# yuliangguo/OmniFusion

Measured on AMD Instinct MI355X. Metric: panoramas/sec at 512x1024 ERP, N=18 256^2 patches; equi2pers+pers2equi GB/s vs HBM peak, higher is better.
Workload: dtype f16x3 (fp16 hi/lo pairs, fp32 accumulate: fp32-class); 1 GPU; cfg2/cfg4 shard: 8 panoramas/GPU/step, 512x1024 ERP, fov 80, nrows 4 (18 patches); full single-pass spherical_fusion forward (confidence=True) at patch size 128 — the only size the reference network exists at (SURVEY 0.1); random-init weights (seed 42); inputs resident in HBM; resample pair at 18x256^2 reported in roofline_resample; per_gpu_batch=8, global_batch=8, parallelism=image-sharded x1, execution=3 forwards in flight per GPU on 3 streams (spherical_fusion.pipelined)

## Files before the change

include/omnifusion.h:

```cpp
#ifndef OMNIFUSION_H_
#define OMNIFUSION_H_

#include <stddef.h>
#include <stdint.h>

#ifdef __cplusplus
extern "C" {
#endif

#define OMNI_VERSION 200

enum omni_status {
    OMNI_OK = 0,
    OMNI_ERR_INVALID = 1,
    OMNI_ERR_HIP = 2,
    OMNI_ERR_UNSUPPORTED = 3
};

enum omni_layout { OMNI_LAYOUT_BCHWN = 0, OMNI_LAYOUT_BNCHW = 1, OMNI_LAYOUT_BNHWC = 2,
                   OMNI_LAYOUT_BCHNW = 3  };
enum omni_dtype { OMNI_F32 = 0, OMNI_F16 = 1 };

typedef void* omni_stream_t;
typedef struct omni_geometry omni_geometry_t;
// ... 42 lines not shown
                       int ph, int pw, int nrows, float fov_h, float fov_w, int layout, omni_stream_t stream);
int omni_pers2equi_bwd(const void* grad_erp, void* grad_pers, int dtype, int B, int C, int ph, int pw,
                       int H, int W, int nrows, float fov_h, float fov_w, int layout, omni_stream_t stream);
int omni_conv2d_nhwc_f32(const float* src1, const float* src2, const float* wt, const float* bias,
                         const float* res, float* dst, int M, int H, int W, int C1, int C2, int Cout,
                         int KH, int KW, int stride, int pad, int act, omni_stream_t stream);
int omni_conv2d_splitk_plan(long long rows, int Cout, int ksteps);
int omni_conv2d_nhwc_f32_ws(const float* src1, const float* src2, const float* wt, const float* bias,
                            const float* res, float* dst, int M, int H, int W, int C1, int C2, int Cout,
                            int KH, int KW, int stride, int pad, int act, int splitk, float* ws, size_t ws_bytes,
                            omni_stream_t stream);
int omni_conv2d_nhwc_f16x3_ws(const float* src1, const float* src2, const void* wt16, const float* bias,
                              const float* res, float* dst, int M, int H, int W, int C1, int C2, int Cout,
                              int KH, int KW, int stride, int pad, int act, int splitk, float* ws, size_t ws_bytes,
                              omni_stream_t stream);
int omni_conv2d_sh_f16x3_ws(const void* src1, const void* src2, const void* wt16, const float* bias,
                            const void* res, void* dst, int fmt, int M, int H, int W, int C1, int C2, int Cout,
                            int KH, int KW, int stride, int pad, int act, int splitk, float* ws, size_t ws_bytes,
                            omni_stream_t stream);
int omni_gemm_rows_sh_f16x3(const void* x, const void* wt16r, const float* bias, const float* res, void* dst, int fmt,
                            int rows, int K, int N, int act, omni_stream_t stream);
int omni_gemm_rows_pack(const void* wt16, void* wt16r, int N, int K, omni_stream_t stream);
int omni_gemm_rows_ln_sh_f16x3(const float* x, const float* ln_weight, const float* ln_bias, float eps, const void* wt16r, const float* bias,
                               const float* res, void* dst, int fmt, int rows, int N, int act, omni_stream_t stream);
int omni_conv3x3_up2_sh_f16x3(const void* src, const void* wt16, const float* bias, void* dst, int fmt,
                              int M, int Hl, int Wl, int C, int Cout, int act, omni_stream_t stream);
size_t omni_up2_heads_scratch_bytes(int M, int P);
int omni_conv3x3_up2_heads_sh_f16x3(const void* src, const void* wt16, const float* bias, const void* heads_w16f, float bias_pred, float bias_weight,
                                    float* scratch, size_t scratch_bytes, float* out_a, float* out_c, int M, int P, int confidence, omni_stream_t stream);
int omni_conv3x3_up2_heads_sh_f16x1(const void* src, const void* wt16, const float* bias, const void* heads_w16f, float bias_pred, float bias_weight,
                                    float* scratch, size_t scratch_bytes, float* out_a, float* out_c, int M, int P, int confidence, omni_stream_t stream);
int omni_heads_pack_f16x3(const float* w_host, void* dst_host);
int omni_conv2d_sh_f16x3_post_ws(const void* src1, const void* src2, const void* wt16, const float* bias,
                                 const void* res, void* dst, int fmt, int M, int H, int W, int C1, int C2, int Cout,
                                 int KH, int KW, int stride, int pad, int act, int splitk, float* ws, size_t ws_bytes,
                                 const float* post, size_t post_elems, omni_stream_t stream);
int omni_wino_input_sh(const void* src, void* V, int M, int H, int W, int C, omni_stream_t stream);
int omni_conv3x3_wino_sh_f16x3(const void* V, const void* wt16, const float* bias, const void* res, void* dst, int fmt,
                               int M, int H, int W, int C, int Cout, int act, int splitk, float* ws, size_t ws_bytes, omni_stream_t stream);
int omni_sh_from_f32(const float* src, void* dst, size_t n, omni_stream_t stream);
int omni_sh_to_f32(const void* src, float* dst, size_t n, omni_stream_t stream);
int omni_sh_overflow(int* flag, int reset);
int omni_stem_f32(const float* src, const float* wt, const float* bias, float* dst, int M, int P, omni_stream_t stream);
int omni_maxpool3x3s2_f32(const float* src, float* dst, int M, int H, int W, int C, omni_stream_t stream);
int omni_upsample_bilinear_f32(const float* src, float* dst, int M, int H, int W, int C, int Ho, int Wo, omni_stream_t stream);
int omni_add_hw_f32(float* x, const float* y, int M, int HW, int C, omni_stream_t stream);
int omni_add_period_f32(float* x, const float* y, size_t total, size_t period, omni_stream_t stream);
int omni_stem_sh(const float* src, const float* wt, const float* bias, void* dst, int M, int P, omni_stream_t stream);
int omni_stem_sh_f16x3(const float* src, const void* wt16, const float* bias, void* dst, int M, int P, omni_stream_t stream);
int omni_stem_sh_f16x1(const float* src, const void* wt16, const float* bias, void* dst, int M, int P, omni_stream_t stream);
int omni_maxpool3x3s2_sh(const void* src, void* dst, int M, int H, int W, int C, omni_stream_t stream);
int omni_upsample_bilinear_sh(const void* src, void* dst, int M, int H, int W, int C, int Ho, int Wo, omni_stream_t stream);
int omni_up2_tapsum_sh(const float* y, const float* bias, void* dst, int M, int Hl, int Wl, int Cout, int act, omni_stream_t stream);
int omni_add_hw_sh(void* x, const float* y, int M, int HW, int C, omni_stream_t stream);
int omni_add_period_sh(void* x, const float* y, size_t total, size_t period, omni_stream_t stream);
int omni_layernorm512_sh(const float* x, const float* g, const float* b, void* y, int rows, float eps, omni_stream_t stream);
int omni_gemm_rows_slices_sh_f16x3(const void* x, const void* wt16r, float* parts, int rows, int K, int N, int slices, omni_stream_t stream);
int omni_gemm_rows_ln_parts_sh_f16x3(const float* parts, int nparts, const float* pbias, const float* pres, float* xout,
                                     const float* ln_weight, const float* ln_bias, float eps, const void* wt16r, const float* bias,
                                     void* dst, int fmt, int rows, int N, int act, omni_stream_t stream);
int omni_splitk_reduce_ln512(const float* parts, int nparts, const float* bias, const float* res, float* tok, const float* ln_weight, const float* ln_bias,
                             float eps, void* y, int fmt, int rows, omni_stream_t stream);
int omni_gemm_sh_f16x3_ln512_ws(const void* x, const void* wt16, const float* bias, const float* res, float* tok, const float* ln_g, const float* ln_b,
                                float eps, void* y, int fmt, int rows, int K, int splitk, float* ws, size_t ws_bytes, omni_stream_t stream);
int omni_attention_qkv_sh(const float* qkv, void* out, int B, int N, omni_stream_t stream);
int omni_token_pack_f32(const float* d, const float* pos, float* tok, int M, int N, int HW, int C, omni_stream_t stream);
int omni_layernorm512_f32(const float* x, const float* g, const float* b, float* y, int rows, float eps, omni_stream_t stream);
int omni_attention_f32(const float* q, const float* kv, float* out, int B, int N, omni_stream_t stream);
int omni_heads_f32(const float* x, const float* w, float bias_pred, float bias_weight, float* out_a, float* out_c,
                   int M, int P, int confidence, omni_stream_t stream);
int omni_mlp_points_f32(const float* xyz, const float* depth, const float* w1, const float* b1, const float* w2,
                        const float* b2, float* out, int Mo, int N, int HW, omni_stream_t stream);

int omni_masked_median_f32(const float* x, const float* mask, size_t n, unsigned* ws, float* out, omni_stream_t stream);
int omni_depth_metrics_f32(float* pred, const float* gt, const float* mask, const float* scale_num, const float* scale_den,
                           size_t n, double* ws, float* out, omni_stream_t stream);

size_t omni_semantic_workspace_bytes(size_t npix);
int omni_semantic_step_f32(const float* logits, const int64_t* target, int B, int C, size_t HW, int64_t ignore_index, int K,
                           void* workspace, float* loss, int64_t* pred, int64_t* confusion, omni_stream_t stream);
int omni_semantic_grad_f32(const float* logits, const int64_t* target, int B, int C, size_t HW, int64_t ignore_index,
                           const void* workspace, const float* grad_out, float* grad_logits, omni_stream_t stream);
int omni_confusion_matrix_i64(const int64_t* pred, const int64_t* gt, size_t n, int K, int64_t* confusion, int64_t* n_bad,
                              omni_stream_t stream);

int omni_preprocess_rgb_u8(const unsigned char* src_hwc, float* dst_chw, int B, int Hs, int Ws, int H, int W, omni_stream_t stream);
int omni_preprocess_depth_u16(const unsigned short* src, float* depth, unsigned char* mask, int B, int Hs, int Ws, int H, int W,
                              float min_depth, float max_depth, omni_stream_t stream);
int omni_png_info(const void* data, size_t nbytes, int* width, int* height, int* bit_depth, int* color_type);
int omni_png_decode(const void* data, size_t nbytes, void* dst, int H, int W, int kind);
int omni_png_decode_batch(const void* const* datas, const size_t* nbytes, void* const* dsts, int n, int H, int W, int kind, int threads);
int omni_zlib_inflate(const void* src, size_t nbytes, void* dst, size_t cap, size_t* produced, size_t* consumed);
int omni_png_checksums(const void* data, size_t nbytes, unsigned* crc32, unsigned* adler32);
size_t omni_berhu_workspace_bytes(int B);
int omni_berhu_loss_f32(const float* pred, const float* gt, const float* mask, const float* weights, int B, size_t per_item,
                        void* workspace, float* loss, omni_stream_t stream);
int omni_berhu_grad_f32(const float* pred, const float* gt, const float* mask, const float* weights, int B, size_t per_item,
                        const void* workspace, const float* grad_out, float* grad_pred, omni_stream_t stream);
int omni_pointcloud_ply_f32(const float* depth, const float* rgb, unsigned char* records, int B, int H, int W, omni_stream_t stream);

size_t omni_dibr_workspace_bytes(int B, int C, int H, int W);
int omni_splat_render_f32(const float* img, const float* depth, const float* coords, float max_depth,
                          float* recon, unsigned char* mask , int B, int C, int H, int W,
                          void* workspace, omni_stream_t stream);
int omni_dibr_f32(const float* img, const float* depth, const float* uvgrid, const float* sgrid, int grid_batched,
                  float baseline, int mode, float* recon, unsigned char* mask ,
// ... 47 lines not shown
```

omnifusion_amd/_lib.py:

```python
import ctypes
import os

_HERE = os.path.dirname(os.path.abspath(__file__))
LIB_PATH = os.environ.get("OMNI_LIB_VARIANT") or os.path.join(_HERE, "csrc", "libomnifusion_hip.so")
LIB_PATH_DEBUG = os.path.join(_HERE, "csrc", "libomnifusion_hip_dbg.so")

OMNI_OK, OMNI_ERR_INVALID, OMNI_ERR_HIP, OMNI_ERR_UNSUPPORTED = 0, 1, 2, 3
LAYOUT_BCHWN, LAYOUT_BNCHW, LAYOUT_BNHWC, LAYOUT_BCHNW = 0, 1, 2, 3
F32, F16 = 0, 1

_lib = None


class OmniLibraryMissing(ImportError):
    pass


EXPORTS = [
    "omni_version", "omni_last_error", "omni_set_option", "omni_get_option", "omni_num_patches", "omni_patch_centers",
    "omni_geometry_create", "omni_geometry_destroy", "omni_geometry_cache_clear", "omni_geometry_cache_size",
    "omni_equi2pers", "omni_equi2pers_aux", "omni_pers2equi", "omni_pers2equi_conf", "omni_patches_to_planar",
    "omni_equi2pers_g", "omni_pers2equi_g", "omni_equi2pers_bwd", "omni_pers2equi_bwd",
    "omni_conv2d_nhwc_f32", "omni_stem_f32", "omni_maxpool3x3s2_f32", "omni_upsample_bilinear_f32",
    "omni_add_hw_f32", "omni_add_period_f32", "omni_token_pack_f32", "omni_layernorm512_f32",
    "omni_attention_f32", "omni_heads_f32", "omni_mlp_points_f32",
    "omni_conv2d_nhwc_f16x3_ws", "omni_conv2d_sh_f16x3_ws", "omni_conv2d_sh_f16x3_post_ws", "omni_gemm_rows_sh_f16x3", "omni_gemm_rows_ln_sh_f16x3", "omni_gemm_rows_pack", "omni_conv3x3_up2_sh_f16x3", "omni_conv3x3_up2_heads_sh_f16x3", "omni_conv3x3_up2_heads_sh_f16x1", "omni_up2_heads_scratch_bytes", "omni_heads_pack_f16x3", "omni_sh_from_f32", "omni_sh_to_f32", "omni_sh_overflow",
    "omni_stem_sh", "omni_stem_sh_f16x3", "omni_stem_sh_f16x1", "omni_maxpool3x3s2_sh", "omni_upsample_bilinear_sh", "omni_up2_tapsum_sh", "omni_add_hw_sh", "omni_add_period_sh", "omni_layernorm512_sh", "omni_gemm_sh_f16x3_ln512_ws", "omni_gemm_rows_slices_sh_f16x3", "omni_gemm_rows_ln_parts_sh_f16x3", "omni_splitk_reduce_ln512", "omni_wino_input_sh", "omni_conv3x3_wino_sh_f16x3", "omni_attention_qkv_sh",
    "omni_conv2d_splitk_plan", "omni_conv2d_nhwc_f32_ws",
    "omni_masked_median_f32", "omni_depth_metrics_f32",
    "omni_png_info", "omni_png_decode", "omni_png_decode_batch", "omni_zlib_inflate", "omni_png_checksums",
    "omni_preprocess_rgb_u8", "omni_preprocess_depth_u16", "omni_berhu_workspace_bytes", "omni_berhu_loss_f32", "omni_berhu_grad_f32",
    "omni_pointcloud_ply_f32",
    "omni_dibr_workspace_bytes", "omni_splat_render_f32", "omni_dibr_f32",
    "omni_splat_render_wt_f32", "omni_dibr_wt_f32", "omni_dibr_bwd_workspace_bytes", "omni_splat_render_bwd_f32", "omni_dibr_bwd_f32",
    "omni_ssim_f32", "omni_photometric_workspace_bytes", "omni_photometric_grad_scratch_bytes", "omni_photometric_loss_f32",
    "omni_photometric_grad_f32",
    "omni_freeview_rotations", "omni_freeview_equi2pers_f32", "omni_freeview_pers2equi_f32", "omni_freeview_merge_f32",
    "omni_freeview_bwd_workspace_bytes", "omni_freeview_equi2pers_bwd_f32", "omni_freeview_pers2equi_bwd_f32", "omni_freeview_merge_bwd_f32",
    "omni_semantic_workspace_bytes", "omni_semantic_step_f32", "omni_semantic_grad_f32", "omni_confusion_matrix_i64",
]


def load():
    global _lib
    if _lib is not None:
        return _lib
    if not os.path.exists(LIB_PATH):
        raise OmniLibraryMissing(
            f"{LIB_PATH} not found: build it with `python -m omnifusion_amd.build` "
            "(hipcc --offload-arch=gfx950).  There is no fallback path.")
    import torch
    lib = ctypes.CDLL(LIB_PATH)
    lib.omni_last_error.restype = ctypes.c_char_p
    lib.omni_version.restype = ctypes.c_int
    lib.omni_up2_heads_scratch_bytes.restype = ctypes.c_size_t
    lib.omni_dibr_workspace_bytes.restype = ctypes.c_size_t
    lib.omni_splat_render_f32.argtypes = [ctypes.c_void_p] * 3 + [ctypes.c_float] + [ctypes.c_void_p] * 2 + [ctypes.c_int] * 4 + [ctypes.c_void_p] * 2
    lib.omni_dibr_f32.argtypes = [ctypes.c_void_p] * 4 + [ctypes.c_int, ctypes.c_float, ctypes.c_int] + [ctypes.c_void_p] * 2 + \
        [ctypes.c_int] * 4 + [ctypes.c_void_p] * 2
    vp, ci, cf = ctypes.c_void_p, ctypes.c_int, ctypes.c_float
    lib.omni_splat_render_wt_f32.argtypes = [vp] * 3 + [cf] + [vp] * 3 + [ci] * 4 + [vp] * 2
    lib.omni_dibr_wt_f32.argtypes = [vp] * 4 + [ci, cf, ci] + [vp] * 3 + [ci] * 4 + [vp] * 2
    lib.omni_dibr_bwd_workspace_bytes.restype = ctypes.c_size_t
    lib.omni_splat_render_bwd_f32.argtypes = [vp] * 6 + [cf] + [vp] * 3 + [ci] * 4 + [vp] * 2
    lib.omni_dibr_bwd_f32.argtypes = [vp] * 7 + [ci, cf, ci] + [vp] * 2 + [ci] * 4 + [vp] * 2
    lib.omni_ssim_f32.argtypes = [vp] * 2 + [ci] * 5 + [vp, ci, vp, vp]
    lib.omni_photometric_workspace_bytes.restype = ctypes.c_size_t
    lib.omni_photometric_grad_scratch_bytes.restype = ctypes.c_size_t
    lib.omni_photometric_loss_f32.argtypes = [vp, vp, vp, ci, vp, ci] + [ci] * 5 + [vp, ci, cf] + [vp] * 3
    lib.omni_photometric_grad_f32.argtypes = [vp, vp, vp, ci, vp, ci] + [ci] * 5 + [vp, ci, cf] + [vp] * 5
    lib.omni_freeview_rotations.argtypes = [vp, vp, ci, vp, vp]
    lib.omni_freeview_equi2pers_f32.argtypes = [vp] * 3 + [ci] * 7 + [cf, cf, ci, vp]
    lib.omni_freeview_pers2equi_f32.argtypes = [vp] * 4 + [ci] * 6 + [cf, cf, vp]
    lib.omni_freeview_merge_f32.argtypes = [vp] * 4 + [ci] * 7 + [cf, cf, vp]
    lib.omni_freeview_bwd_workspace_bytes.restype = ctypes.c_size_t
    lib.omni_freeview_bwd_workspace_bytes.argtypes = [ci] * 5
    lib.omni_freeview_equi2pers_bwd_f32.argtypes = [vp] * 3 + [ci] * 7 + [cf, cf, ci, vp, vp]
    lib.omni_freeview_pers2equi_bwd_f32.argtypes = [vp] * 3 + [ci] * 6 + [cf, cf, vp, vp]
    lib.omni_freeview_merge_bwd_f32.argtypes = [vp] * 3 + [ci] * 7 + [cf, cf, vp, vp]
    sz, i64 = ctypes.c_size_t, ctypes.c_int64
# ... 63 lines not shown
```

omnifusion_amd/csrc/omni_conv_sh.hip:

```cpp
#include "omni_conv_sh_common.h"

namespace {

__constant__ float wino_coef[16][4] = {
    {1, 0, 0, 0}, {1, 1, 0, 0}, {1, -1, 0, 0}, {0, -1, 0, 0},
    {1, 0, 1, 0}, {1, 1, 1, 1}, {1, -1, 1, -1}, {0, -1, 0, -1},
    {1, 0, -1, 0}, {1, 1, -1, -1}, {1, -1, -1, 1}, {0, -1, 0, 1},
    {0, 0, -1, 0}, {0, 0, -1, -1}, {0, 0, -1, 1}, {0, 0, 0, 1}};
template <int BM, int BN, int WM, int WN, int NST = 3, int NL = 0, bool PP = false, bool WINO = false, bool X1 = false>
__global__ __launch_bounds__(64 * (WM * WN + NL)) void conv_sh_kernel(ShConvArgs a)
{
    static_assert(!(WINO && X1), "Winograd: f16x3 only");
    static_assert(!PP || (NL > 0 && WM * WN == 8 && NST >= 3), "ping-pong: eight matrix waves (two per SIMD) + loader waves, three stages");
    static_assert(!WINO || (PP && BM / WM == 32 && BN / WN == 32), "Winograd: the ping-pong kernel with 32 x 32 wave tiles");
    constexpr int NW = WM * WN, LW = NL > 0 ? NL : NW, RPP = 8 * LW;
    constexpr int TM = BM / WM / 32, TN = BN / WN / 32;
    constexpr int APASS = BM / RPP, BPASS = BN / RPP, LPS = APASS + BPASS;
    static_assert(APASS >= 1 && BPASS >= 1, "a tile side must cover at least one DMA pass");
    constexpr int A_BYTES = BM * 128, STAGE = (BM + BN) * 128;
    __shared__ __attribute__((aligned(1024))) unsigned char lds[NST * STAGE];
    __shared__ long long cst[OMNI_ABL(32768) ? 256 : 1];
    const bool stamped = OMNI_ABL(32768) && blockIdx.x == 0 && blockIdx.y == 0 && a.ws != nullptr && a.splitk <= 1;
    auto cstamp = [&](int k) { if (OMNI_ABL(32768) && stamped && (threadIdx.x & 63) == 0 && k < 256) cst[k] = clock64(); };
    auto cdump = [&]() { if (OMNI_ABL(32768) && stamped && threadIdx.x == 0) for (int i = 0; i < 256; ++i) reinterpret_cast<long long*>(a.ws)[i] = cst[i]; };
// ... 602 lines not shown
    const long long rows = (long long)M * a.Ho * a.Wo;
    if (rows <= 0 || rows >= (1ll << 31) || (long long)M * H * W >= (1ll << 31))
        OMNI_FAIL(OMNI_ERR_UNSUPPORTED, "omni_conv2d_sh: too many pixels for 32-bit row indices");
    a.rows = (int)rows;
    const int ksteps = KH * KW * ((C1 + C2) / 32);
    if ((long long)M * H * W * (C1 > C2 ? C1 : C2) * 4 >= (1ll << 31) || (long long)Cout * ksteps * 128 >= (1ll << 31))
        OMNI_FAIL(OMNI_ERR_UNSUPPORTED, "omni_conv2d_sh: an operand of 2 GiB or more (32-bit buffer offsets)");
    int S = splitk;
    if (S > ksteps) S = ksteps;
    if (S > 1 && (!ws || ws_bytes < (size_t)S * rows * Cout * sizeof(float)))
        OMNI_FAIL(OMNI_ERR_INVALID, "omni_conv2d_sh: split-K workspace too small");
    a.splitk = S > 1 ? S : 1; a.ws = ws;
    a.wt_major = omni_options().conv_wt_major == 2 || (omni_options().conv_wt_major == 1 &&
                 (long long)Cout * ksteps * 128 > (long long)M * H * W * (C1 + C2) * 4) ? 1 : 0;
    a.post = post; a.post_rows = 1; a.wino_th = a.wino_tw = a.wino_pix = 0;
    if (post) {
        if (Cout <= 0 || post_elems == 0 || post_elems % (size_t)Cout || post_elems / (size_t)Cout > 0x7fffffffull)
            OMNI_FAIL(OMNI_ERR_INVALID, "omni_conv2d_sh: the post-activation addend must hold whole rows of Cout channels");
        if (a.splitk > 1) OMNI_FAIL(OMNI_ERR_UNSUPPORTED, "omni_conv2d_sh: no post-activation addend with split-K");
        a.post_rows = (unsigned)(post_elems / (size_t)Cout);
    }
    hipStream_t s = (hipStream_t)stream;
    if (fmt & 8) conv_sh_select<true>(a, fmt, s);
    else         conv_sh_select<false>(a, fmt, s);
    OMNI_HIP(hipGetLastError());
    if (a.splitk > 1 && reduce) {
        const size_t n4 = (size_t)rows * Cout / 4;
        hipLaunchKernelGGL(sh_splitk_reduce_kernel, dim3((unsigned)((n4 + 255) / 256)), dim3(256), 0, s, (const float*)ws, bias, res, dst,
                           n4, Cout, a.splitk, (size_t)rows * Cout, act, a.dst_sh, a.res_f32);
        OMNI_HIP(hipGetLastError());
    }
    return OMNI_OK;
}

extern "C" int omni_splitk_reduce_ln512(const float* parts, int nparts, const float* bias, const float* res, float* tok, const float* lg, const float* lb,
                                        float eps, void* y, int fmt, int rows, omni_stream_t stream)
{
    if (!parts || nparts < 1 || !tok || !lg || !lb || !y || rows <= 0) OMNI_FAIL(OMNI_ERR_INVALID, "omni_splitk_reduce_ln512: null pointer or empty input");
    hipStream_t s = (hipStream_t)stream;
    if (fmt & 1) hipLaunchKernelGGL(sh_splitk_reduce_ln512_kernel<true>, dim3((rows + 3) / 4), dim3(256), 0, s, parts, bias, res, tok, lg, lb, y, rows, nparts, (size_t)rows * 512, eps);
    else         hipLaunchKernelGGL(sh_splitk_reduce_ln512_kernel<false>, dim3((rows + 3) / 4), dim3(256), 0, s, parts, bias, res, tok, lg, lb, y, rows, nparts, (size_t)rows * 512, eps);
    OMNI_HIP(hipGetLastError());
    return OMNI_OK;
}

OMNI_SH_OVERFLOW_ACCESSOR(omni_sh_overflow_conv)

extern "C" int omni_sh_overflow(int* flag, int reset)
{
    if (!flag) OMNI_FAIL(OMNI_ERR_INVALID, "omni_sh_overflow: null output");
    OMNI_HIP(hipDeviceSynchronize());
    unsigned v = 0;
    if (omni_sh_overflow_conv(&v, reset) != 0 || omni_sh_overflow_halo(&v, reset) != 0 || omni_sh_overflow_up2(&v, reset) != 0 ||
        omni_sh_overflow_rows(&v, reset) != 0 || omni_sh_overflow_net(&v, reset) != 0)
        OMNI_FAIL(OMNI_ERR_HIP, "omni_sh_overflow: could not read the device flag");
    *flag = v ? 1 : 0;
    return OMNI_OK;
}

extern "C" int omni_sh_from_f32(const float* src, void* dst, size_t n, omni_stream_t stream)
{
    if (!src || !dst || n % 32) OMNI_FAIL(OMNI_ERR_INVALID, "omni_sh_from_f32: null pointer or n % 32 != 0");
    if (n == 0) return OMNI_OK;
    hipLaunchKernelGGL(sh_from_f32_kernel, dim3((unsigned)((n / 4 + 255) / 256)), dim3(256), 0, (hipStream_t)stream, src, dst, n / 4);
    OMNI_HIP(hipGetLastError());
    return OMNI_OK;
}
extern "C" int omni_sh_to_f32(const void* src, float* dst, size_t n, omni_stream_t stream)
{
    if (!src || !dst || n % 32) OMNI_FAIL(OMNI_ERR_INVALID, "omni_sh_to_f32: null pointer or n % 32 != 0");
    if (n == 0) return OMNI_OK;
    hipLaunchKernelGGL(sh_to_f32_kernel, dim3((unsigned)((n / 4 + 255) / 256)), dim3(256), 0, (hipStream_t)stream, src, dst, n / 4);
    OMNI_HIP(hipGetLastError());
    return OMNI_OK;
}

namespace {

__global__ __launch_bounds__(256) void wino_input_sh_kernel(const void* __restrict__ src, void* __restrict__ V, int M, int H, int W, int C, size_t nt)
{
    const size_t i = (size_t)blockIdx.x * 256 + threadIdx.x;
    const int cq = C >> 2;
    if (i >= nt * cq) return;
    const size_t tl = i / cq;
    const int c = (int)(i - tl * cq) * 4;
    const int tw = W >> 1, th = H >> 1;
    const int m = (int)(tl / (size_t)(th * tw)), rem = (int)(tl - (size_t)m * th * tw), ty = rem / tw, tx = rem - ty * tw;
    f4v d[4][4];
#pragma unroll
    for (int a_ = 0; a_ < 4; ++a_)
#pragma unroll
        for (int b_ = 0; b_ < 4; ++b_) {
            const int y = 2 * ty - 1 + a_, x = 2 * tx - 1 + b_;
            d[a_][b_] = ((unsigned)y < (unsigned)H && (unsigned)x < (unsigned)W) ? act_load4<true>(src, (((size_t)m * H + y) * W + x) * C + c) : (f4v)(0.0f);
        }
    f4v u[4][4];
#pragma unroll
    for (int b_ = 0; b_ < 4; ++b_) { u[0][b_] = d[0][b_] - d[2][b_]; u[1][b_] = d[1][b_] + d[2][b_]; u[2][b_] = d[2][b_] - d[1][b_]; u[3][b_] = d[1][b_] - d[3][b_]; }
#pragma unroll
    for (int xi = 0; xi < 4; ++xi) {
        const f4v v0 = u[xi][0] - u[xi][2], v1 = u[xi][1] + u[xi][2], v2 = u[xi][2] - u[xi][1], v3 = u[xi][1] - u[xi][3];
        act_store4<true>(V, ((size_t)(4 * xi + 0) * nt + tl) * C + c, v0);
        act_store4<true>(V, ((size_t)(4 * xi + 1) * nt + tl) * C + c, v1);
        act_store4<true>(V, ((size_t)(4 * xi + 2) * nt + tl) * C + c, v2);
        act_store4<true>(V, ((size_t)(4 * xi + 3) * nt + tl) * C + c, v3);
    }
}
// ... 43 lines not shown
```

omnifusion_amd/csrc/omni_conv_sh_common.h:

```cpp
#pragma once
#include <stdlib.h>
#include <algorithm>
#include <type_traits>
#include "omni_internal.h"
#include "omni_sh.h"

#ifndef OMNI_CONV_ABL
#define OMNI_CONV_ABL 0
#endif
#define OMNI_ABL(bit) ((OMNI_CONV_ABL & (bit)) != 0)
#ifndef OMNI_PP_PRIO
#define OMNI_PP_PRIO 0
#endif
#ifndef OMNI_G1_PW
#define OMNI_G1_PW 4
#endif

namespace {

typedef float f16v __attribute__((ext_vector_type(16)));
typedef float f4v __attribute__((ext_vector_type(4)));
typedef _Float16 h8v __attribute__((ext_vector_type(8)));
typedef _Float16 h4v __attribute__((ext_vector_type(4)));
typedef _Float16 h2v __attribute__((ext_vector_type(2)));
// ... 150 lines not shown
#pragma unroll
                for (int e = 0; e < 4; ++e) { v0[e] += fmaf((float)rl[kk][e], 4.8828125e-4f, (float)rh[kk][e]); v1[e] += fmaf((float)rl[kk][4 + e], 4.8828125e-4f, (float)rh[kk][4 + e]); }
            }
            if (a.act == OMNI_ACT_RELU) {
#pragma unroll
                for (int e = 0; e < 4; ++e) { v0[e] = fmaxf(v0[e], 0.f); v1[e] = fmaxf(v1[e], 0.f); }
            } else if (a.act == OMNI_ACT_GELU) {
#pragma unroll
                for (int e = 0; e < 4; ++e) { v0[e] = 0.5f * v0[e] * (1.0f + erff(v0[e] * 0.70710678118654752440f)); v1[e] = 0.5f * v1[e] * (1.0f + erff(v1[e] * 0.70710678118654752440f)); }
            }
            if (post) { v0 += pa[kk]; v1 += pb[kk]; }
            h4v h0, l0, h1, l1;
            sh_split4(v0, h0, l0); sh_split4(v1, h1, l1);
            h8v oh, ol;
#pragma unroll
            for (int e = 0; e < 4; ++e) { oh[e] = h0[e]; oh[4 + e] = h1[e]; ol[e] = l0[e]; ol[4 + e] = l1[e]; }
            *reinterpret_cast<h8v*>((unsigned char*)a.dst + off[kk]) = oh;
            *reinterpret_cast<h8v*>((unsigned char*)a.dst + off[kk] + 64) = ol;
        }
    }
}

__device__ __forceinline__ void splitk_finish(f4v v, size_t o, const float* __restrict__ bias, const void* __restrict__ res, void* __restrict__ dst,
                                              int Cout, int act, int dst_sh, int res_f32)
{
    if (bias) v += *reinterpret_cast<const f4v*>(bias + (o % Cout));
    if (res && res_f32) v += *reinterpret_cast<const f4v*>((const float*)res + o);
    else if (res) {
        const unsigned char* rp = (const unsigned char*)res + sh_off(o);
        v += sh_join4(*reinterpret_cast<const h4v*>(rp), *reinterpret_cast<const h4v*>(rp + 64));
    }
    if (act == OMNI_ACT_RELU) { v.x = fmaxf(v.x, 0.f); v.y = fmaxf(v.y, 0.f); v.z = fmaxf(v.z, 0.f); v.w = fmaxf(v.w, 0.f); }
    else if (act == OMNI_ACT_GELU) {
#pragma unroll
        for (int e = 0; e < 4; ++e) v[e] = 0.5f * v[e] * (1.0f + erff(v[e] * 0.70710678118654752440f));
    }
    if (dst_sh) {
        h4v hi, lo; sh_split4(v, hi, lo);
        unsigned char* dp = (unsigned char*)dst + sh_off(o);
        *reinterpret_cast<h4v*>(dp) = hi; *reinterpret_cast<h4v*>(dp + 64) = lo;
    } else {
        *reinterpret_cast<f4v*>((float*)dst + o) = v;
    }
}

constexpr int HT_W = 32, HPW = HT_W + 2;

}

void omni_halo_launch(const void* args, int bn, int th, bool up2, int iw, bool x1, unsigned grid, hipStream_t s);
int omni_sh_overflow_halo(unsigned* out, int reset);
int omni_sh_overflow_up2(unsigned* out, int reset);
int omni_sh_overflow_rows(unsigned* out, int reset);
int omni_sh_overflow_net(unsigned* out, int reset);
```

omnifusion_amd/isa.py:

```python
import os
import re
import subprocess
import sys
import tempfile

LLVM = os.environ.get("OMNI_LLVM_BIN", "/opt/rocm/lib/llvm/bin")
TARGET = "hipv4-amdgcn-amd-amdhsa--gfx950"
FORBIDDEN = re.compile(r"\bv_pk_(mul|add|fma)_f32\b")
COUNTED = ("e2p_box_kernel", "p2e_lds_kernel", "p2e_walk_kernel", "e2p_ref_kernel")
HOT = ("conv_sh_kernel", "conv3x3_halo_sh_kernel", "conv3x3_up2_g1_kernel", "stem_f16x3_pc_kernel", "heads_kernel", "maxpool_kernel",
       "layernorm512_kernel", "attention_kernel", "upsample_sh8_kernel")
HOST_ONLY = ("omni_png.o", "omni_geometry.o")


def _device_object(obj, tmp):
    fat = os.path.join(tmp, "fat.bin")
    co = os.path.join(tmp, "dev.co")
    r = subprocess.run([os.path.join(LLVM, "llvm-objcopy"), "--dump-section", f".hip_fatbin={fat}", obj, os.path.join(tmp, "copy.o")],
                       stderr=subprocess.DEVNULL)
    if r.returncode != 0 or not os.path.exists(fat) or os.path.getsize(fat) == 0:
        return None
    subprocess.check_call([os.path.join(LLVM, "clang-offload-bundler"), "--unbundle", "--type=o", f"--input={fat}",
                           f"--targets={TARGET}", f"--output={co}"])
    return co


def disassemble(obj):
    with tempfile.TemporaryDirectory() as tmp:
        co = _device_object(obj, tmp)
        if co is None:
            return ""
        return subprocess.check_output([os.path.join(LLVM, "llvm-objdump"), "-d", "--mcpu=gfx950", co]).decode()


def kernel_meta(obj):
    with tempfile.TemporaryDirectory() as tmp:
        co = _device_object(obj, tmp)
        if co is None:
            return []
        txt = subprocess.check_output([os.path.join(LLVM, "llvm-readelf"), "--notes", co]).decode()
    out, cur = [], None
    keys = {".vgpr_count": "vgpr", ".agpr_count": "agpr", ".sgpr_count": "sgpr", ".group_segment_fixed_size": "lds",
            ".private_segment_fixed_size": "scratch", ".vgpr_spill_count": "vgpr_spill", ".sgpr_spill_count": "sgpr_spill",
            ".name": "name"}
    for line in txt.splitlines():
        m = re.match(r"^  - \.(\w+):\s*(\S+)\s*$", line)
        if m:
            cur = {}
            out.append(cur)
            line = "    ." + m.group(1) + ": " + m.group(2)
        m = re.match(r"^    (\.\w+):\s*(\S+)\s*$", line)
        if m and cur is not None and m.group(1) in keys:
            v = m.group(2)
            cur[keys[m.group(1)]] = v if m.group(1) == ".name" else int(v)
    return [k for k in out if "name" in k]


def demangle(names):
    try:
        p = subprocess.run([os.path.join(LLVM, "llvm-cxxfilt")], input="\n".join(names).encode(), stdout=subprocess.PIPE, check=True)
        return p.stdout.decode().splitlines()
    except Exception:
        return list(names)

# ... 68 lines not shown
```

omnifusion_amd/model/_engine.py:

```python
import ctypes
import os

import torch

from .. import _lib
from ..equi_pers.equi2pers_v3 import equi2pers_patches, equi2pers_aux, pair, _NPATCH
from ..equi_pers.pers2equi_v3 import pers2equi, pers2equi_conf

ACT_NONE, ACT_RELU, ACT_GELU = 0, 1, 2
_LAYERS = [("layer1", 3, 1), ("layer2", 4, 2), ("layer3", 6, 2), ("layer4", 3, 2)]
_BN_EPS = 1e-5
PRECISIONS = ("f16x3", "f16x1", "fp32")


def _p(t):
    return ctypes.c_void_p(t.data_ptr()) if t is not None else None


def split_weights_f16x3(w):
    w = w.to(torch.float32)
    wmax = float(w.abs().max()) if w.numel() else 0.0
    if not wmax < 65504.0:
        raise ValueError(f"folded weight magnitude {wmax:g} is outside the fp16 range of the f16x3 operand format: "
                         "run this checkpoint with OMNI_NET_PRECISION=fp32")
# ... 239 lines not shown
        _lib.check(rc, "gemm+ln " + w16key)
        return out, y, None

    def _ln_gemm_parts(self, pending, lnw, lnb, eps, w16key, rows, Nout):
        parts, S, bkey, res_tok = pending
        tok = torch.empty((rows, 512), dtype=torch.float32, device=parts.device)
        out = torch.empty((rows, Nout), dtype=torch.float32, device=parts.device)
        rc = _lib.load().omni_gemm_rows_ln_parts_sh_f16x3(_p(parts), S, _p(self.w[bkey]), _p(res_tok), _p(tok), _p(self.w[lnw]), _p(self.w[lnb]), ctypes.c_float(eps),
                                                          _p(self._rows_weights(w16key, Nout, 512)), None, _p(out), 0, rows, Nout, ACT_NONE, self._s)
        _lib.check(rc, "ln+gemm (slices) " + w16key)
        return tok, out

    fuse_ln = os.environ.get("OMNI_FUSE_LN", "1") != "0"

    def _ln_gemm_sh(self, x, lnw, lnb, eps, w16key, bkey, rows, Nout, act=ACT_NONE, out_sh=False):
        if self._bs == 1 and self.latency_plan and self.rows_gemm and self.fuse_ln and rows <= 32:
            lib = _lib.load()
            out = torch.empty((rows, Nout), dtype=torch.float32, device=x.device)
            _lib.check(lib.omni_gemm_rows_ln_sh_f16x3(_p(x), _p(self.w[lnw]), _p(self.w[lnb]), ctypes.c_float(eps), _p(self._rows_weights(w16key, Nout, 512)),
                                                      _p(self.w[bkey]) if bkey else None, None, _p(out), 1 if out_sh else 0, rows, Nout, act, self._s), "ln+gemm " + w16key)
            return out
        return self._gemm_sh(self._ln_sh(x, lnw, lnb, rows, eps), w16key, bkey, rows, 512, Nout, act=act, out_sh=out_sh)

    def _ln_sh(self, x, wk, bk, rows, eps):
        y = torch.empty_like(x)
        _lib.check(_lib.load().omni_layernorm512_sh(_p(x), _p(self.w[wk]), _p(self.w[bk]), _p(y), rows, ctypes.c_float(eps), self._s), "layernorm")
        return y

    def _ln(self, x, wk, bk, rows, eps):
        y = torch.empty_like(x)
        _lib.check(_lib.load().omni_layernorm512_f32(_p(x), _p(self.w[wk]), _p(self.w[bk]), _p(y), rows, ctypes.c_float(eps), self._s), "layernorm")
        return y

    def _up(self, x, M, H, Wd, C, Ho, Wo):
        y = torch.empty((M, Ho, Wo, C), dtype=torch.float32, device=x.device)
        fn = _lib.load().omni_upsample_bilinear_sh if self.sh else _lib.load().omni_upsample_bilinear_f32
        _lib.check(fn(_p(x), _p(y), M, H, Wd, C, Ho, Wo, self._s), "upsample")
        return y

    fold_point_feat = True
    fuse_up = True

    def _up_conv(self, x, key, M, H, Wd, C, Cout, act, out_f32=False, out=None):
        Ho, Wo = 2 * H, 2 * Wd
        if self.sh and self.fuse_up and Wo % 32 == 0 and Ho % 4 == 0:
            if out is None:
                out = torch.empty((M, Ho, Wo, Cout), dtype=torch.float32, device=x.device)
            _lib.check(_lib.load().omni_conv3x3_up2_sh_f16x3(_p(x), _p(self.w[key + ".w16"]), _p(self.w[key + ".b"]), _p(out),
                                                             (0 if out_f32 else 1) | (4 if (self._bs == 1 and self.latency_plan) else 0) | self._x1,
                                                             M, H, Wd, C, Cout, act, self._s), "up+conv " + key)
            return out
        return self._conv(self._up(x, M, H, Wd, C, Ho, Wo), key, M, Ho, Wo, C, Cout, 3, 1, 1, act, out_f32=out_f32, out=out)

    taps_first = frozenset(("de_conv0_0",))

    def _up_conv_taps(self, x, key, M, H, Wd, C, Cout, act):
        if key in self.taps_first and self.sh and self.terms == 3 and Cout % 32 == 0 and H * Wd <= 64:
            y = self._conv(x, key + ".taps", M, H, Wd, C, 9 * Cout, 1, 1, 0, ACT_NONE, bias=False, out_f32=True)
            out = torch.empty((M, 2 * H, 2 * Wd, Cout), dtype=torch.float32, device=x.device)
            _lib.check(_lib.load().omni_up2_tapsum_sh(_p(y), _p(self.w[key + ".b"]), _p(out), M, H, Wd, Cout, act, self._s), "tap sum " + key)
            return out
        return self._conv(self._up(x, M, H, Wd, C, 2 * H, 2 * Wd), key, M, 2 * H, 2 * Wd, C, Cout, 3, 1, 1, act)

    def transformer(self, d, bs):
        lib = _lib.load()
        dev = d.device
        self._s = ctypes.c_void_p(torch.cuda.current_stream(dev).cuda_stream)
        self._bs = bs
        N, P32 = self.npatches, self.patch_size[0] // 32
        M = bs * N
        sh = self.sh
        new = lambda *s: torch.empty(s, dtype=torch.float32, device=dev)
        tok = new(M, 512)
        _lib.check(lib.omni_token_pack_f32(_p(d), _p(self.w["pos"]), _p(tok), M, N, P32 * P32, 32, self._s), "token_pack")
        normed = None
        pending = None
        for i in range(6):
            t = f"t{i}."
            if sh:
                if pending is not None:
                    tok, qkv = self._ln_gemm_parts(pending, t + "norm1.weight", t + "norm1.bias", 1e-5, t + "attn.qkv.w16", M, 1536)
                    pending = None
                elif normed is not None:
                    qkv = self._gemm_sh(normed, t + "attn.qkv.w16", None, M, 512, 1536)
                else:
                    qkv = self._ln_gemm_sh(tok, t + "norm1.weight", t + "norm1.bias", 1e-5, t + "attn.qkv.w16", None, M, 1536)
                att = new(M, 512)
                _lib.check(lib.omni_attention_qkv_sh(_p(qkv), _p(att), bs, N, self._s), "attention")
                tok = self._gemm_sh(att, t + "attn.proj.w16", t + "attn.proj.bias", M, 512, 512, res=tok)
                h = self._ln_gemm_sh(tok, t + "norm2.weight", t + "norm2.bias", 1e-5, t + "mlp.fc1.w16", t + "mlp.fc1.bias", M, 2048, act=ACT_GELU, out_sh=True)
                nxt = (f"t{i + 1}.norm1.weight", f"t{i + 1}.norm1.bias", 1e-5, True) if i < 5 else ("enc_norm.w", "enc_norm.b", 1e-6, False)
                tok, normed, pending = self._fc2_ln(h, t + "mlp.fc2.w16", t + "mlp.fc2.bias", M, tok, nxt)
                continue
            y = self._ln(tok, t + "norm1.weight", t + "norm1.bias", M, 1e-5)
            q = self._gemm(y, t + "attn.q.weight", None, M, 512, 512)
            kv = self._gemm(y, t + "attn.kv.weight", None, M, 512, 1024)
            att = new(M, 512)
            _lib.check(lib.omni_attention_f32(_p(q), _p(kv), _p(att), bs, N, self._s), "attention")
            tok = self._gemm(att, t + "attn.proj.weight", t + "attn.proj.bias", M, 512, 512, res=tok)
            y = self._ln(tok, t + "norm2.weight", t + "norm2.bias", M, 1e-5)
            h = self._gemm(y, t + "mlp.fc1.weight", t + "mlp.fc1.bias", M, 512, 2048, act=ACT_GELU)
            tok = self._gemm(h, t + "mlp.fc2.weight", t + "mlp.fc2.bias", M, 2048, 512, res=tok)
        if sh and pending is not None:
            parts, S, bkey, res_tok = pending
            tok_sum, tok = new(M, 512), new(M, 512)
            _lib.check(lib.omni_splitk_reduce_ln512(_p(parts), S, _p(self.w[bkey]), _p(res_tok), _p(tok_sum), _p(self.w["enc_norm.w"]), _p(self.w["enc_norm.b"]),
                                                    ctypes.c_float(1e-6), _p(tok), 0, M, self._s), "reduce+ln")
        else:
            tok = normed if (sh and normed is not None) else self._ln(tok, "enc_norm.w", "enc_norm.b", M, 1e-6)
        return tok
# ... 113 lines not shown
```

Baseline: 4137 panoramas/s.

## Fuse tap GEMM and upsample tap-sum into one kernel for decoder up-convs

Adds a fused kernel that computes the 1x1 tap GEMM (9*Cout slab per block) with MFMA f16x3 into LDS, then performs the bilinear-upsample tap summation, bias and ReLU directly from LDS. This removes the fp32 intermediate tap tensor round trip through HBM and one kernel launch. It also extends the taps-first path to de_conv1_0. The trade-off is a larger LDS footprint, warp-specialized loader/compute waves, and a restriction to small low-res spatial sizes (Hl*Wl<=64).

```diff
diff --git a/include/omnifusion.h b/include/omnifusion.h
--- a/include/omnifusion.h
+++ b/include/omnifusion.h
@@ -118,6 +118,8 @@
 int omni_maxpool3x3s2_sh(const void* src, void* dst, int M, int H, int W, int C, omni_stream_t stream);
 int omni_upsample_bilinear_sh(const void* src, void* dst, int M, int H, int W, int C, int Ho, int Wo, omni_stream_t stream);
 int omni_up2_tapsum_sh(const float* y, const float* bias, void* dst, int M, int Hl, int Wl, int Cout, int act, omni_stream_t stream);
+int omni_up2_taps_sh_f16x3(const void* src, const void* wt16_taps, const float* bias, void* dst,
+                           int M, int Hl, int Wl, int C, int Cout, int act, omni_stream_t stream);
 int omni_add_hw_sh(void* x, const float* y, int M, int HW, int C, omni_stream_t stream);
 int omni_add_period_sh(void* x, const float* y, size_t total, size_t period, omni_stream_t stream);
 int omni_layernorm512_sh(const float* x, const float* g, const float* b, void* y, int rows, float eps, omni_stream_t stream);
diff --git a/omnifusion_amd/_lib.py b/omnifusion_amd/_lib.py
--- a/omnifusion_amd/_lib.py
+++ b/omnifusion_amd/_lib.py
@@ -25,7 +25,7 @@
     "omni_add_hw_f32", "omni_add_period_f32", "omni_token_pack_f32", "omni_layernorm512_f32",
     "omni_attention_f32", "omni_heads_f32", "omni_mlp_points_f32",
     "omni_conv2d_nhwc_f16x3_ws", "omni_conv2d_sh_f16x3_ws", "omni_conv2d_sh_f16x3_post_ws", "omni_gemm_rows_sh_f16x3", "omni_gemm_rows_ln_sh_f16x3", "omni_gemm_rows_pack", "omni_conv3x3_up2_sh_f16x3", "omni_conv3x3_up2_heads_sh_f16x3", "omni_conv3x3_up2_heads_sh_f16x1", "omni_up2_heads_scratch_bytes", "omni_heads_pack_f16x3", "omni_sh_from_f32", "omni_sh_to_f32", "omni_sh_overflow",
-    "omni_stem_sh", "omni_stem_sh_f16x3", "omni_stem_sh_f16x1", "omni_maxpool3x3s2_sh", "omni_upsample_bilinear_sh", "omni_up2_tapsum_sh", "omni_add_hw_sh", "omni_add_period_sh", "omni_layernorm512_sh", "omni_gemm_sh_f16x3_ln512_ws", "omni_gemm_rows_slices_sh_f16x3", "omni_gemm_rows_ln_parts_sh_f16x3", "omni_splitk_reduce_ln512", "omni_wino_input_sh", "omni_conv3x3_wino_sh_f16x3", "omni_attention_qkv_sh",
+    "omni_stem_sh", "omni_stem_sh_f16x3", "omni_stem_sh_f16x1", "omni_maxpool3x3s2_sh", "omni_upsample_bilinear_sh", "omni_up2_tapsum_sh", "omni_up2_taps_sh_f16x3", "omni_add_hw_sh", "omni_add_period_sh", "omni_layernorm512_sh", "omni_gemm_sh_f16x3_ln512_ws", "omni_gemm_rows_slices_sh_f16x3", "omni_gemm_rows_ln_parts_sh_f16x3", "omni_splitk_reduce_ln512", "omni_wino_input_sh", "omni_conv3x3_wino_sh_f16x3", "omni_attention_qkv_sh",
     "omni_conv2d_splitk_plan", "omni_conv2d_nhwc_f32_ws",
     "omni_masked_median_f32", "omni_depth_metrics_f32",
     "omni_png_info", "omni_png_decode", "omni_png_decode_batch", "omni_zlib_inflate", "omni_png_checksums",
diff --git a/omnifusion_amd/csrc/omni_conv_sh.hip b/omnifusion_amd/csrc/omni_conv_sh.hip
--- a/omnifusion_amd/csrc/omni_conv_sh.hip
+++ b/omnifusion_amd/csrc/omni_conv_sh.hip
@@ -678,7 +678,7 @@
     OMNI_HIP(hipDeviceSynchronize());
     unsigned v = 0;
     if (omni_sh_overflow_conv(&v, reset) != 0 || omni_sh_overflow_halo(&v, reset) != 0 || omni_sh_overflow_up2(&v, reset) != 0 ||
-        omni_sh_overflow_rows(&v, reset) != 0 || omni_sh_overflow_net(&v, reset) != 0)
+        omni_sh_overflow_rows(&v, reset) != 0 || omni_sh_overflow_net(&v, reset) != 0 || omni_sh_overflow_taps(&v, reset) != 0)
         OMNI_FAIL(OMNI_ERR_HIP, "omni_sh_overflow: could not read the device flag");
     *flag = v ? 1 : 0;
     return OMNI_OK;
diff --git a/omnifusion_amd/csrc/omni_conv_sh_common.h b/omnifusion_amd/csrc/omni_conv_sh_common.h
--- a/omnifusion_amd/csrc/omni_conv_sh_common.h
+++ b/omnifusion_amd/csrc/omni_conv_sh_common.h
@@ -226,4 +226,5 @@
 int omni_sh_overflow_halo(unsigned* out, int reset);
 int omni_sh_overflow_up2(unsigned* out, int reset);
 int omni_sh_overflow_rows(unsigned* out, int reset);
+int omni_sh_overflow_taps(unsigned* out, int reset);
 int omni_sh_overflow_net(unsigned* out, int reset);
diff --git a/omnifusion_amd/csrc/omni_conv_taps.hip b/omnifusion_amd/csrc/omni_conv_taps.hip
--- /dev/null
+++ b/omnifusion_amd/csrc/omni_conv_taps.hip
@@ -0,0 +1,190 @@
+#include "omni_conv_sh_common.h"
+
+namespace {
+
+constexpr int TF_ROWS = 64, TF_SLAB = 32, TF_TAPS = 9, TF_BN = TF_TAPS * TF_SLAB, TF_PITCH = TF_BN;
+constexpr int TF_NST = 3, TF_A_BYTES = TF_ROWS * 128, TF_STAGE = (TF_ROWS + TF_BN) * 128;
+constexpr int TF_MW = 6, TF_LW = 4;
+constexpr int TF_APW = TF_ROWS / 8 / TF_LW, TF_BPW = TF_BN / 8 / TF_LW, TF_LPS = TF_APW + TF_BPW;
+static_assert(TF_ROWS * TF_PITCH * 4 <= TF_NST * TF_STAGE, "the slab aliases the operand stages");
+static_assert((TF_NST - 1) * TF_LPS <= 63, "vmcnt is a 6-bit counter");
+
+__global__ __launch_bounds__(64 * (TF_MW + TF_LW)) void up2_taps_fused_kernel(const void* __restrict__ src, const void* __restrict__ wt, const float* __restrict__ bias,
+                                                                             void* __restrict__ dst, int M, int Hl, int Wl, int C, int Cout, int act)
+{
+    __shared__ __attribute__((aligned(1024))) unsigned char lds[TF_NST * TF_STAGE];
+    const int t = threadIdx.x, lane = t & 63;
+    const int wave = __builtin_amdgcn_readfirstlane(t >> 6);
+    const int HW = Hl * Wl, ipb = TF_ROWS / HW, ng = Cout >> 5;
+    const unsigned lb = omni_xcd_remap(blockIdx.x, gridDim.x);
+    const int bm = (int)(lb / (unsigned)ng), c0 = (int)(lb % (unsigned)ng) * TF_SLAB;
+    const int img0 = bm * ipb, nimg = min(ipb, M - img0);
+    const int ksteps = C >> 5;
+    const int wm = wave / 3, wn = wave - 3 * wm;
+    f16v acc[3], acc1[3];
+#pragma unroll
+    for (int j = 0; j < 3; ++j) { acc[j] = (f16v)(0.0f); acc1[j] = (f16v)(0.0f); }
+
+    if (wave >= TF_MW) {
+        const int lw = wave - TF_MW;
+        const rsrc_t rsa = make_rsrc(src, (size_t)M * HW * C * 4);
+        const rsrc_t rsw = make_rsrc(wt, (size_t)TF_TAPS * Cout * ksteps * 128);
+        int voa[TF_APW], vob[TF_BPW];
+#pragma unroll
+        for (int i = 0; i < TF_APW; ++i) {
+            const int d = 4 * (lw + TF_LW * i) + (lane >> 4), g = (lane & 15) ^ (d & 15), r = 2 * d + (g >> 3);
+            voa[i] = r < nimg * HW ? (img0 * HW + r) * C * 4 + (g & 7) * 16 : (int)0x80000000;
+        }
+#pragma unroll
+        for (int i = 0; i < TF_BPW; ++i) {
+            const int d = 4 * (lw + TF_LW * i) + (lane >> 4), g = (lane & 15) ^ (d & 15), n = 2 * d + (g >> 3);
+            vob[i] = ((n >> 5) * Cout + c0 + (n & 31)) * ksteps * 128 + (g & 7) * 16;
+        }
+        auto issue = [&](int ks, int slot) {
+            unsigned char* sb = lds + slot * TF_STAGE + lw * 1024;
+#pragma unroll
+            for (int i = 0; i < TF_APW; ++i) dma16(rsa, sb + i * (1024 * TF_LW), voa[i], ks * 128);
+#pragma unroll
+            for (int i = 0; i < TF_BPW; ++i) dma16(rsw, sb + TF_A_BYTES + i * (1024 * TF_LW), vob[i], ks * 128);
+        };
+#pragma unroll
+        for (int s = 0; s < TF_NST - 1; ++s)
+            if (s < ksteps) issue(s, s);
+        int slot = TF_NST - 1;
+        for (int ks = 0; ks < ksteps; ++ks) {
+            if (ks + TF_NST - 2 < ksteps) wait_vm<(TF_NST - 2) * TF_LPS>();
+            else                          wait_vm<0>();
+            __builtin_amdgcn_s_barrier();
+            asm volatile("" ::: "memory");
+            if (ks + TF_NST - 1 < ksteps) issue(ks + TF_NST - 1, slot);
+            slot = slot + 1 == TF_NST ? 0 : slot + 1;
+        }
+    } else {
+        int foa[4], fob[4];
+        {
+            const int r = lane & 31, v = r >> 1, h = lane >> 5;
+#pragma unroll
+            for (int k = 0; k < 4; ++k) {
+                const int f = v * 256 + ((((r & 1) * 8 + 2 * k + h) ^ v) * 16);
+                foa[k] = f + wm * 32 * 128;
+                fob[k] = f + TF_A_BYTES + wn * 96 * 128;
+            }
+        }
+        int slot = 0;
+        for (int ks = 0; ks < ksteps; ++ks) {
+            wait_lds_reads();
+            __builtin_amdgcn_s_barrier();
+            asm volatile("" ::: "memory");
+            const unsigned char* sl = lds + slot * TF_STAGE;
+            h8v ah[2], al[2], bh[2][3], bl[2][3];
+#pragma unroll
+            for (int kc = 0; kc < 2; ++kc) {
+                ah[kc] = *reinterpret_cast<const h8v*>(sl + foa[kc]);
+                al[kc] = *reinterpret_cast<const h8v*>(sl + foa[2 + kc]);
+#pragma unroll
+                for (int j = 0; j < 3; ++j) {
+                    bh[kc][j] = *reinterpret_cast<const h8v*>(sl + j * 4096 + fob[kc]);
+                    bl[kc][j] = *reinterpret_cast<const h8v*>(sl + j * 4096 + fob[2 + kc]);
+                }
+            }
+#pragma unroll
+            for (int kc = 0; kc < 2; ++kc)
+#pragma unroll
+                for (int j = 0; j < 3; ++j) {
+                    acc[j] = __builtin_amdgcn_mfma_f32_32x32x16_f16(bh[kc][j], ah[kc], acc[j], 0, 0, 0);
+                    acc1[j] = __builtin_amdgcn_mfma_f32_32x32x16_f16(bl[kc][j], ah[kc], acc1[j], 0, 0, 0);
+                    acc1[j] = __builtin_amdgcn_mfma_f32_32x32x16_f16(bh[kc][j], al[kc], acc1[j], 0, 0, 0);
+                }
+            slot = slot + 1 == TF_NST ? 0 : slot + 1;
+        }
+    }
+    wait_lds_reads();
+    __syncthreads();
+    if (wave < TF_MW) {
+        const int sr = lane & 3;
+        float* slab = reinterpret_cast<float*>(lds) + (wm * 32 + (lane & 31)) * TF_PITCH + wn * 96 + 4 * (lane >> 5);
+#pragma unroll
+        for (int j = 0; j < 3; ++j) {
+            f4v v[4], r1[4];
+#pragma unroll
+            for (int q = 0; q < 4; ++q)
+#pragma unroll
+                for (int e = 0; e < 4; ++e) v[q][e] = acc_join<false>(acc1[j][4 * q + e], acc[j][4 * q + e]);
+#pragma unroll
+            for (int i = 0; i < 4; ++i)
+#pragma unroll
+                for (int e = 0; e < 4; ++e) r1[i][e] = (sr & 1) ? v[(i + 1) & 3][e] : v[i][e];
+#pragma unroll
+            for (int i = 0; i < 4; ++i) {
+                f4v w;
+#pragma unroll
+                for (int e = 0; e < 4; ++e) w[e] = (sr & 2) ? r1[(i + 2) & 3][e] : r1[i][e];
+                *reinterpret_cast<f4v*>(slab + 32 * j + 8 * ((i + sr) & 3)) = w;
+            }
+        }
+    }
+    __syncthreads();
+
+    const float* ts_all = reinterpret_cast<const float*>(lds);
+    const int Ho = 2 * Hl, Wo = 2 * Wl, NP = Ho * Wo, total = nimg * NP;
+    const int pi = ((lane >> 5) << 2) | ((0x31130220u >> (((lane >> 2) & 7) * 4)) & 3);
+    const int q = (lane & 7) * 4;
+    f4v bv = (f4v)(0.0f);
+    if (bias) bv = *reinterpret_cast<const f4v*>(bias + c0 + q);
+    for (int pp = wave * 8 + pi; pp < total; pp += 8 * (TF_MW + TF_LW)) {
+        const int im = pp / NP, p = pp - im * NP;
+        const float* ts_img = ts_all + im * HW * TF_PITCH;
+        const int oy = p / Wo, ox = p - oy * Wo;
+        int yo0[3], yo1[3], xo0[3], xo1[3];
+        float ly[3], lx[3];
+        bool vy[3], vx[3];
+#pragma unroll
+        for (int k = 0; k < 3; ++k) {
+            const int py = oy + k - 1, px = ox + k - 1;
+            vy[k] = (unsigned)py < (unsigned)Ho; vx[k] = (unsigned)px < (unsigned)Wo;
+            const float fy = fmaxf(0.5f * ((float)py + 0.5f) - 0.5f, 0.0f), fx = fmaxf(0.5f * ((float)px + 0.5f) - 0.5f, 0.0f);
+            const int y0 = (int)fy, x0 = (int)fx;
+            ly[k] = fy - (float)y0; lx[k] = fx - (float)x0;
+            yo0[k] = y0 * Wl * TF_PITCH; yo1[k] = (y0 + (y0 < Hl - 1 ? 1 : 0)) * Wl * TF_PITCH;
+            xo0[k] = x0 * TF_PITCH;      xo1[k] = (x0 + (x0 < Wl - 1 ? 1 : 0)) * TF_PITCH;
+        }
+        f4v acc = (f4v)(0.0f);
+#pragma unroll
+        for (int ky = 0; ky < 3; ++ky)
+#pragma unroll
+            for (int kx = 0; kx < 3; ++kx) {
+                if (!(vy[ky] && vx[kx])) continue;
+                const float* b = ts_img + (ky * 3 + kx) * TF_SLAB + q;
+                const f4v v00 = *reinterpret_cast<const f4v*>(b + yo0[ky] + xo0[kx]), v01 = *reinterpret_cast<const f4v*>(b + yo0[ky] + xo1[kx]);
+                const f4v v10 = *reinterpret_cast<const f4v*>(b + yo1[ky] + xo0[kx]), v11 = *reinterpret_cast<const f4v*>(b + yo1[ky] + xo1[kx]);
+                const float hy = 1.0f - ly[ky], hx = 1.0f - lx[kx];
+                const float w00 = hy * hx, w01 = hy * lx[kx], w10 = ly[ky] * hx, w11 = ly[ky] * lx[kx];
+#pragma unroll
+                for (int e = 0; e < 4; ++e) acc[e] = fmaf(w11, v11[e], fmaf(w10, v10[e], fmaf(w01, v01[e], fmaf(w00, v00[e], acc[e]))));
+            }
+        f4v o = acc + bv;
+        if (act == OMNI_ACT_RELU) { o.x = fmaxf(o.x, 0.f); o.y = fmaxf(o.y, 0.f); o.z = fmaxf(o.z, 0.f); o.w = fmaxf(o.w, 0.f); }
+        act_store4<true>(dst, (((size_t)(img0 + im) * Ho + oy) * Wo + ox) * Cout + c0 + q, o);
+    }
+}
+
+}
+
+OMNI_SH_OVERFLOW_ACCESSOR(omni_sh_overflow_taps)
+
+extern "C" int omni_up2_taps_sh_f16x3(const void* src, const void* wt16_taps, const float* bias, void* dst,
+                                      int M, int Hl, int Wl, int C, int Cout, int act, omni_stream_t stream)
+{
+    if (!src || !wt16_taps || !dst || M < 1 || Hl < 1 || Wl < 1 || C < 1 || Cout < 1) OMNI_FAIL(OMNI_ERR_INVALID, "omni_up2_taps_sh_f16x3: null tensor or empty shape");
+    if ((uintptr_t)src % 16 || (uintptr_t)wt16_taps % 16 || (uintptr_t)bias % 16 || (uintptr_t)dst % 16)
+        OMNI_FAIL(OMNI_ERR_INVALID, "omni_up2_taps_sh_f16x3: tensors must be 16-byte aligned");
+    if (C % 32 || Cout % TF_SLAB || (long long)Hl * Wl > TF_ROWS || (act != OMNI_ACT_NONE && act != OMNI_ACT_RELU))
+        OMNI_FAIL(OMNI_ERR_UNSUPPORTED, "omni_up2_taps_sh_f16x3: C % 32 == 0, Cout % 32 == 0, Hl * Wl <= 64, no activation or ReLU");
+    const int HW = Hl * Wl, ipb = TF_ROWS / HW;
+    const long long blocks = ((long long)M + ipb - 1) / ipb * (Cout / TF_SLAB);
+    if ((long long)M * HW * C * 4 >= (1ll << 31) || (long long)TF_TAPS * Cout * C * 4 >= (1ll << 31) || blocks >= (1ll << 31))
+        OMNI_FAIL(OMNI_ERR_UNSUPPORTED, "omni_up2_taps_sh_f16x3: an operand of 2 GiB or more (32-bit buffer offsets)");
+    hipLaunchKernelGGL(up2_taps_fused_kernel, dim3((unsigned)blocks), dim3(64 * (TF_MW + TF_LW)), 0, (hipStream_t)stream, src, wt16_taps, bias, dst, M, Hl, Wl, C, Cout, act);
+    OMNI_HIP(hipGetLastError());
+    return OMNI_OK;
+}
diff --git a/omnifusion_amd/isa.py b/omnifusion_amd/isa.py
--- a/omnifusion_amd/isa.py
+++ b/omnifusion_amd/isa.py
@@ -9,7 +9,7 @@
 FORBIDDEN = re.compile(r"\bv_pk_(mul|add|fma)_f32\b")
 COUNTED = ("e2p_box_kernel", "p2e_lds_kernel", "p2e_walk_kernel", "e2p_ref_kernel")
 HOT = ("conv_sh_kernel", "conv3x3_halo_sh_kernel", "conv3x3_up2_g1_kernel", "stem_f16x3_pc_kernel", "heads_kernel", "maxpool_kernel",
-       "layernorm512_kernel", "attention_kernel", "upsample_sh8_kernel")
+       "layernorm512_kernel", "attention_kernel", "upsample_sh8_kernel", "up2_taps_fused_kernel")
 HOST_ONLY = ("omni_png.o", "omni_geometry.o")
 
 
diff --git a/omnifusion_amd/model/_engine.py b/omnifusion_amd/model/_engine.py
--- a/omnifusion_amd/model/_engine.py
+++ b/omnifusion_amd/model/_engine.py
@@ -315,10 +315,17 @@
             return out
         return self._conv(self._up(x, M, H, Wd, C, Ho, Wo), key, M, Ho, Wo, C, Cout, 3, 1, 1, act, out_f32=out_f32, out=out)
 
-    taps_first = frozenset(("de_conv0_0",))
+    taps_first = frozenset(("de_conv0_0", "de_conv1_0"))
+    taps_fused = True
 
     def _up_conv_taps(self, x, key, M, H, Wd, C, Cout, act):
         if key in self.taps_first and self.sh and self.terms == 3 and Cout % 32 == 0 and H * Wd <= 64:
+            if self.taps_fused and C % 32 == 0:
+                out = torch.empty((M, 2 * H, 2 * Wd, Cout), dtype=torch.float32, device=x.device)
+                rc = _lib.load().omni_up2_taps_sh_f16x3(_p(x), _p(self.w[key + ".taps.w16"]), _p(self.w[key + ".b"]), _p(out), M, H, Wd, C, Cout, act, self._s)
+                if rc != _lib.OMNI_ERR_UNSUPPORTED:
+                    _lib.check(rc, "taps " + key)
+                    return out
             y = self._conv(x, key + ".taps", M, H, Wd, C, 9 * Cout, 1, 1, 0, ACT_NONE, bias=False, out_f32=True)
             out = torch.empty((M, 2 * H, 2 * Wd, Cout), dtype=torch.float32, device=x.device)
             _lib.check(_lib.load().omni_up2_tapsum_sh(_p(y), _p(self.w[key + ".b"]), _p(out), M, H, Wd, Cout, act, self._s), "tap sum " + key)
```

Measured after the change: 4151 panoramas/s, median of 6. About the same (+0.3%).
